# radixsorth/PorousFreezeThaw

Hardware: AMD Instinct MI355X
Metric: Mcells·RK-steps/s at 400³ grid, 1/2/4/8 MI355X; % HBM roofline (higher is better)
Workload: dtype f64; 1 GPU; 400^3 default Params: 200x200x400 cells, Z-slab split 1-way (200x200x400 on rank 0); grid_nodes=400, literal_cube=False, calc_mode=0, cells=16000000, parallelism=zslab1, gl_static=False, kz=auto, tile=1, recompute=True, accepted_steps_total=2981, self_exchange=False, service_callback=False, gl_store_skipped=True, pair_kernels=True, gated_steps=0, gate_misses=0

## Files before the change

porousfreezethaw_amd/csrc/pft_kernels.hip:

```cpp
#include "pft_slab.h"

#include "pft_cosh.h"
#include "pft_ic_ops.h"
#include "pft_tanh.h"

#pragma clang fp contract(off)

__thread char g_err[256];

int fail(hipError_t e, const char* what)
{
  snprintf(g_err, sizeof(g_err), "%s: %s", what, hipGetErrorString(e));
  (void)hipGetLastError();
  return -(int)e - 1000;
}


struct Col {
  double c, xm, xp, ym, yp, zm, zp;
};

__device__ __forceinline__ double lam_of(const pft_consts& c, double p, double g)
{
  return g * c.lam_g + (1.0 - g) * (p * c.lam_i + (1.0 - p) * c.lam_w);
// ... 430 lines not shown

template <int STAGE, int MODE, bool GLS>
__global__ __launch_bounds__(PFT_BLOCK) void merson_stage(StageArgs a, pft_consts c)
{
  const int lin = xcd_remap(blockIdx.x, a.ntile * a.nchunk);
  const int tile = lin % a.ntile, chunk = lin / a.ntile;
  const int cell = tile * PFT_BLOCK + threadIdx.x;
  const bool active = cell < a.plane;
  const int cc = active ? cell : a.plane - 1;
  const int j = cc / a.n1, i = cc - j * a.n1;
  const int kb = a.k_begin + chunk * a.kz;
  const int ke = min(kb + a.kspan, a.k_end);

  const int oxm = i > 0 ? -1 : 0, oxp = i < a.n1 - 1 ? 1 : 0;
  const int oym = j > 0 ? -a.n1 : 0, oyp = j < a.n2 - 1 ? a.n1 : 0;

  const double* fin[3] = {a.in, a.in + a.fs, GLS ? a.x + 2 * a.fs : a.in + 2 * a.fs};

  double m = 0.0;
  bool nf = false;
  double zm[3], zc[3], zp[3], zn[3], nb[3][4], nn[3][4];
  if (kb < ke) {
    const long o0 = (long)(kb + 1) * a.plane + cc;
#pragma unroll
    for (int q = 0; q < 3; ++q) {
      zc[q] = fin[q][o0];
      zm[q] = (kb == 0 && !a.has_below) ? zc[q] : fin[q][o0 - a.plane];
      zp[q] = (kb == a.n3 - 1 && !a.has_above) ? zc[q] : fin[q][o0 + a.plane];
      nb[q][0] = fin[q][o0 + oxm];
      nb[q][1] = fin[q][o0 + oxp];
      nb[q][2] = fin[q][o0 + oym];
      nb[q][3] = fin[q][o0 + oyp];
    }
  }
  for (int k = kb; k < ke; ++k) {
    const long o = (long)(k + 1) * a.plane + cc;
    const bool top = (k == a.n3 - 1) && !a.has_above;
    double xv[3], k1v[3], k3v[3], k4v[3];
    if (STAGE >= 1) {
#pragma unroll
      for (int q = 0; q < 3; ++q) {
        if (GLS && q == 2) continue;
        xv[q] = a.x[q * a.fs + o];
        if (STAGE >= 2) k1v[q] = a.k1[q * a.fs + o];
        if (STAGE >= 4) k3v[q] = a.k3[q * a.fs + o];
        if (STAGE >= 5) k4v[q] = a.k4[q * a.fs + o];
      }
    }
    if (k + 1 < ke) {
      const long o1 = o + a.plane;
      const bool top2 = (k + 1 == a.n3 - 1) && !a.has_above;
#pragma unroll
      for (int q = 0; q < 3; ++q) {
        nn[q][0] = fin[q][o1 + oxm];
        nn[q][1] = fin[q][o1 + oxp];
        nn[q][2] = fin[q][o1 + oym];
        nn[q][3] = fin[q][o1 + oyp];
        zn[q] = top2 ? 0.0 : fin[q][o1 + a.plane];
      }
    }
    Col col[3];
#pragma unroll
    for (int q = 0; q < 3; ++q) {
      col[q].c = zc[q];
      col[q].xm = nb[q][0];
      col[q].xp = nb[q][1];
      col[q].ym = nb[q][2];
      col[q].yp = nb[q][3];
      col[q].zm = zm[q];
      col[q].zp = top ? zc[q] : zp[q];
    }
    if (top) col[0].zp = a.T_top;
    double du = 0.0, dp = 0.0;
    const double un = a.noise ? zc[0] + a.noise[(long)k * a.plane + cc] : zc[0];
    rhs_cell<MODE>(c, col[0], col[1], col[2], un, du, dp);
    if (active) {
      if (STAGE == 0) {
        a.kout[o] = du;
        a.kout[a.fs + o] = dp;
        a.kout[2 * a.fs + o] = 0.0;
      } else {
#pragma unroll
        for (int q = 0; q < 3; ++q) {
          if (GLS && q == 2) continue;
          const double K = q == 0 ? du : (q == 1 ? dp : 0.0);
          const long e = q * a.fs + o;
          if (STAGE == 1) {
            a.kout[e] = K;
            a.out[e] = K * a.coef + xv[q];
          } else if (STAGE == 2) {
            a.out[e] = (k1v[q] + K) * a.coef + xv[q];
          } else if (STAGE == 3) {
            a.kout[e] = K;
            a.out[e] = (k1v[q] + 3.0 * K) * a.coef + xv[q];
          } else if (STAGE == 4) {
            a.kout[e] = K;
            a.out[e] = (0.5 * k1v[q] - 1.5 * k3v[q] + 2.0 * K) * a.h + xv[q];
          } else if (STAGE == 5) {
            const double em = q == 0 ? a.em0 : (q == 1 ? a.em1 : a.em2);
            const double ev = em * fabs(0.2 * k1v[q] - 0.9 * k3v[q] + 0.8 * k4v[q] - 0.1 * K);
            if (ev > m) m = ev;
            nf |= !isfinite(ev);
            a.out[e] = xv[q] + a.coef * (0.5 * (k1v[q] + K) + 2.0 * k4v[q]);
          }
        }
      }
    }
#pragma unroll
    for (int q = 0; q < 3; ++q) {
      zm[q] = zc[q];
      zc[q] = zp[q];
      zp[q] = zn[q];
#pragma unroll
      for (int d = 0; d < 4; ++d) nb[q][d] = nn[q][d];
    }
  }

  if (STAGE == 5) {
    __shared__ double red[PFT_BLOCK / 64];
    __shared__ int rnf[PFT_BLOCK / 64];
#pragma unroll
    for (int off = 32; off > 0; off >>= 1) {
      const double o = __shfl_xor(m, off, 64);
      if (o > m) m = o;
    }
    const int anynf = __any(nf);
    const int w = threadIdx.x >> 6;
    if ((threadIdx.x & 63) == 0) {
      red[w] = m;
      rnf[w] = anynf;
    }
    __syncthreads();
    if (threadIdx.x == 0) {
      double bm = red[0];
      int bnf = rnf[0];
      for (int k = 1; k < PFT_BLOCK / 64; ++k) {
        if (red[k] > bm) bm = red[k];
        bnf |= rnf[k];
      }
      if (bm > 0.0) atomicMax(a.eps_bits, (unsigned long long)__double_as_longlong(bm));
      if (bnf) atomicOr(a.nonfinite, 1u);
    }
  }
}


typedef double dbl2 __attribute__((ext_vector_type(2)));

#define PFT_FUSED_LF 680

__device__ __forceinline__ dbl2 ld2(const double* p) { return *reinterpret_cast<const dbl2*>(p); }
__device__ __forceinline__ void st2(double* p, dbl2 v) { *reinterpret_cast<dbl2*>(p) = v; }


struct Ops {
  dbl2 x, k1, k2, k3, k4;
};

template <int STAGE, bool GLS>
__device__ __forceinline__ void load_ops(const StageArgs& a, int q, long o, Ops& r)
{
  r.x = ld2(a.x + q * a.fs + o);
  if (GLS && q == 2) return;
  if (q == 2) {
    constexpr dbl2 z = {0.0, 0.0};
    r.k1 = z; r.k2 = z; r.k3 = z; r.k4 = z;
    return;
  }
  if (STAGE >= 2 && STAGE != 3) r.k1 = ld2(a.k1 + q * a.fs + o);
  if (STAGE == 3) r.k2 = ld2(a.k2 + q * a.fs + o);
  if (STAGE >= 4) r.k3 = ld2(a.k3 + q * a.fs + o);
  if (STAGE == 5) r.k4 = ld2(a.k4 + q * a.fs + o);
}

template <int STAGE, bool GLS>
__device__ __forceinline__ dbl2 stage_in(const StageArgs& a, int q, const Ops& r)
{
  if (STAGE <= 1 || (GLS && q == 2)) return r.x;
  dbl2 v;
#pragma unroll
  for (int s = 0; s < 2; ++s) {
    if (STAGE == 2) v[s] = r.k1[s] * a.cin + r.x[s];
    if (STAGE == 3) v[s] = r.k2[s] * a.cin + r.x[s];
    if (STAGE == 4) v[s] = (r.k1[s] + 3.0 * r.k3[s]) * a.cin + r.x[s];
    if (STAGE == 5) v[s] = (0.5 * r.k1[s] - 1.5 * r.k3[s] + 2.0 * r.k4[s]) * a.cin + r.x[s];
  }
  return v;
}

template <bool GLS>
__device__ __forceinline__ void keep5(int q, const Ops& r, dbl2& x, dbl2& k1, dbl2& k4, dbl2& E)
{
  x = r.x;
  if (q == 2) return;
  k1 = r.k1;
  k4 = r.k4;
#pragma unroll
  for (int s = 0; s < 2; ++s) E[s] = 0.2 * r.k1[s] - 0.9 * r.k3[s] + 0.8 * r.k4[s];
}

template <int STAGE, int MODE, bool GLS>
__global__ __launch_bounds__(PFT_FBLOCK) __attribute__((amdgpu_waves_per_eu(STAGE >= 1 ? 2 : 3))) void merson_fused(StageArgs a, pft_consts c)
{
  const int WX = a.gwx, TY = a.gty, TX = 2 * WX, LW = TX + 4, LH = TY + 2, NH = LW + 2 * TY;
  __shared__ __attribute__((aligned(16))) double lds[2][3][PFT_FUSED_LF];

  unsigned long long gw0 = 0, gw1 = 0, gw2 = 0;
  if (a.gate) {
    gw0 = __hip_atomic_load(a.gate, __ATOMIC_RELAXED, __HIP_MEMORY_SCOPE_AGENT);
    gw1 = a.gate[1];
    gw2 = a.gate[2];
  }
  if (STAGE == 1 && (a.npart > 0 || a.gdev) && (int)blockIdx.x == a.nbw + a.nint) {
    unsigned long long m = 0, f = 0;
    if (a.npart > 0) eps_part_load(a.part, a.npart, m, f);
    if (a.gate) {
      if (gw0 != a.gseq) return;
      a.dt = __longlong_as_double((long long)gw1);
      a.dh = __longlong_as_double((long long)gw2);
    }
    if (a.npart > 0) eps_part_publish(m, f, a.pub, &m, &f);
    if (a.gdev && threadIdx.x == 0) gate_decide(a, a.dt, a.dh, m, (int)f, a.npart > 0);
    return;
  }
  const int ntx = (a.n1 + TX - 1) / TX;
  const bool bw = (int)blockIdx.x < a.nbw;
  const int lin = bw ? xcd_remap(blockIdx.x, a.nbw) : xcd_remap(blockIdx.x - a.nbw, a.nint);
  const int tile = lin % a.ntile, cq = lin / a.ntile;
  const int chunk = bw ? (a.bends ? (cq ? a.nchunk - 1 : 0) : cq) : a.c0 + cq;
  const bool bshort = bw && !a.bends;
  const int x0 = (tile % ntx) * TX, y0 = (tile / ntx) * TY;
  const int tt = min((int)threadIdx.x, WX * TY - 1);
  const int tx = tt % WX, ty = tt / WX;
  const int i0 = x0 + 2 * tx, j = y0 + ty;
  const bool active = (i0 < a.n1) && (j < a.n2) && (int)threadIdx.x < WX * TY;
  const long po = (long)(j < a.n2 ? j : a.n2 - 1) * a.n1 + (i0 < a.n1 ? i0 : a.n1 - 2);
  const int kb = bshort ? chunk * (a.n3 - 2) : a.k_begin + chunk * a.kz;
  const int ke = bshort ? kb + 2 : min(kb + a.kspan, a.k_end);
  const int lo = (ty + 1) * LW + 2 + 2 * tx;

  const int t = threadIdx.x;
  const bool hact = t < 3 * NH;
  const int hf = hact ? t / NH : 0, h = hact ? t % NH : 0;
  int hr, hcp;
  if (h < LW / 2) { hr = 0; hcp = h; }
  else if (h < LW) { hr = LH - 1; hcp = h - LW / 2; }
  else { const int q = h - LW; hr = 1 + q / 2; hcp = (q & 1) ? LW / 2 - 1 : 0; }
  const int hi = x0 - 2 + 2 * hcp, hj = y0 + hr - 1;
  const long hp = (long)(hj < 0 ? 0 : (hj >= a.n2 ? a.n2 - 1 : hj)) * a.n1 +
                  (hi < 0 ? 0 : (hi >= a.n1 ? a.n1 - 2 : hi));
  const int hl = hr * LW + 2 * hcp;
  const int xma = i0 - 2 < 0 ? 1 : 0, xpa = i0 + 2 >= a.n1 ? 1 : 0;

  double m = 0.0;
  bool nf = false;
  dbl2 zm[3], zc[3], zp[3];
  constexpr bool FLUX = MODE != 10 && MODE != 11;
  constexpr bool DEEP = STAGE >= 1 && STAGE <= 4;
  Ops pn[3], ph;
  FaceT fz[2];
  constexpr bool SUM2 = STAGE == 2;
  dbl2 s2c[3], s2n[3];
  dbl2 cx[3], ck1[3], ck4[3], cE[3], nx[3], nk1[3], nk4[3], nE[3];
  int cur = 0;
  const long o0 = (long)(kb + 1) * a.plane + po;
  const bool wlo = kb == 0 && !a.has_below;
  const long ob = wlo ? o0 : o0 - a.plane;
  Ops cop[3], bop[3], hop;
  if (kb < ke) {
#pragma unroll
    for (int q = 0; q < 3; ++q) load_ops<STAGE, GLS>(a, q, o0, cop[q]);
#pragma unroll
    for (int q = 0; q < 3; ++q) load_ops<STAGE, GLS>(a, q, ob, bop[q]);
    load_ops<STAGE, GLS>(a, hf, (long)(kb + 1) * a.plane + hp, hop);
  }
  if (a.gate) {
    if (gw0 != a.gseq) return;
    const double gt = __longlong_as_double((long long)gw1), gh = __longlong_as_double((long long)gw2);
    gate_scalars<STAGE>(a, c, gt, gh);
    a.dt = gt;
    a.dh = gh;
  }
  if (kb < ke) {
#pragma unroll
    for (int q = 0; q < 3; ++q) {
      zc[q] = stage_in<STAGE, GLS>(a, q, cop[q]);
      if constexpr (SUM2) s2c[q] = cop[q].k1;
      if (STAGE == 5) keep5<GLS>(q, cop[q], cx[q], ck1[q], ck4[q], cE[q]);
      zm[q] = wlo ? zc[q] : stage_in<STAGE, GLS>(a, q, bop[q]);
      st2(&lds[0][q][lo], zc[q]);
    }
    if (hact) st2(&lds[0][hf][hl], stage_in<STAGE, GLS>(a, hf, hop));
    if constexpr (DEEP) {
      if (!((kb == a.n3 - 1) && !a.has_above)) {
#pragma unroll
        for (int q = 0; q < 3; ++q) load_ops<STAGE, GLS>(a, q, o0 + a.plane, pn[q]);
      }
      if (hact && kb + 1 < ke) load_ops<STAGE, GLS>(a, hf, (long)(kb + 2) * a.plane + hp, ph);
    }
#pragma unroll
    for (int s = 0; s < 2; ++s)
      fz[s] = face_of(c, zm[1][s], zm[2][s], zm[0][s], zc[1][s], zc[2][s], zc[0][s], FLUX);
    __syncthreads();
  }
  for (int k = kb; k < ke; ++k) {
    const long o = (long)(k + 1) * a.plane + po;
    const bool top = (k == a.n3 - 1) && !a.has_above;
    const bool more = k + 1 < ke;
    if (!top) {
#pragma unroll
      for (int q = 0; q < 3; ++q) {
        if constexpr (DEEP) {
          zp[q] = stage_in<STAGE, GLS>(a, q, pn[q]);
          if constexpr (SUM2) s2n[q] = pn[q].k1;
        } else {
          Ops nop;
          load_ops<STAGE, GLS>(a, q, o + a.plane, nop);
          zp[q] = stage_in<STAGE, GLS>(a, q, nop);
          if constexpr (SUM2) s2n[q] = nop.k1;
          if (STAGE == 5) keep5<GLS>(q, nop, nx[q], nk1[q], nk4[q], nE[q]);
        }
      }
    }
    dbl2 hv = {0.0, 0.0};
    if (more) {
#pragma unroll
      for (int q = 0; q < 3; ++q) st2(&lds[cur ^ 1][q][lo], zp[q]);
      if (hact) {
        if constexpr (DEEP) {
          hv = stage_in<STAGE, GLS>(a, hf, ph);
        } else {
          Ops tmp;
          load_ops<STAGE, GLS>(a, hf, (long)(k + 2) * a.plane + hp, tmp);
          hv = stage_in<STAGE, GLS>(a, hf, tmp);
        }
      }
    }
    if constexpr (DEEP) {
      if (more) {
        if (!((k + 1 == a.n3 - 1) && !a.has_above)) {
#pragma unroll
          for (int q = 0; q < 3; ++q) load_ops<STAGE, GLS>(a, q, o + 2 * a.plane, pn[q]);
        }
        if (hact && k + 2 < ke) load_ops<STAGE, GLS>(a, hf, (long)(k + 3) * a.plane + hp, ph);
      }
    }
    if (top) {
#pragma unroll
      for (int q = 1; q < 3; ++q) zp[q] = zc[q];
      zp[0] = dbl2{a.T_top, a.T_top};
    }
    double du[2], dp[2];
    FaceT fx;
    dbl2 ym2[3], yp2[3];
#pragma unroll
    for (int q = 0; q < 3; ++q) {
      ym2[q] = ld2(&lds[cur][q][lo - LW]);
      yp2[q] = ld2(&lds[cur][q][lo + LW]);
    }
#pragma unroll
    for (int s = 0; s < 2; ++s) {
      Col col[3];
#pragma unroll
      for (int q = 0; q < 3; ++q) {
        const double* L = lds[cur][q];
        const double cen = zc[q][s];
        col[q].c = cen;
        col[q].xm = s == 0 ? L[lo - 1 - xma] : zc[q][0];
        col[q].xp = s == 0 ? zc[q][1] : L[lo + 2 + xpa];
        col[q].ym = ym2[q][s];
        col[q].yp = yp2[q][s];
        col[q].zm = zm[q][s];
        col[q].zp = zp[q][s];
      }
      const double un = a.noise ? zc[0][s] + a.noise[(long)k * a.plane + po + s] : zc[0][s];
      const FaceT fxm =
          s == 0 ? face_of(c, col[1].xm, col[2].xm, col[0].xm, col[1].c, col[2].c, col[0].c, FLUX) : fx;
      FaceT fzp;
      rhs_cell_f<MODE>(c, col[0], col[1], col[2], un, fxm, fz[s], fx, fzp, du[s], dp[s]);
      fz[s] = fzp;
    }
    if (more && hact) st2(&lds[cur ^ 1][hf][hl], hv);
    if (active) {
#pragma unroll
      for (int q = 0; q < 3; ++q) {
        if (q == 2 && STAGE != 0 && (GLS || STAGE <= 4)) continue;
        const dbl2 K = q == 0 ? dbl2{du[0], du[1]} : (q == 1 ? dbl2{dp[0], dp[1]} : dbl2{0.0, 0.0});
        const long e = q * a.fs + o;
        if (SUM2) {
          dbl2 S;
          const dbl2 k1c = s2c[q];
#pragma unroll
          for (int s = 0; s < 2; ++s) S[s] = k1c[s] + K[s];
          st2(a.kout + e, S);
        } else if (STAGE <= 4) {
          st2(a.kout + e, K);
        } else {
          constexpr dbl2 zero2 = {0.0, 0.0};
          const bool z2 = q == 2;
          const dbl2 ox = cx[q], ok1 = z2 ? zero2 : ck1[q], ok4 = z2 ? zero2 : ck4[q];
          dbl2 oE = cE[q];
          if (z2) {
#pragma unroll
            for (int s = 0; s < 2; ++s) oE[s] = 0.2 * 0.0 - 0.9 * 0.0 + 0.8 * 0.0;
          }
          dbl2 r;
#pragma unroll
          for (int s = 0; s < 2; ++s) {
            const double em = q == 0 ? a.em0 : (q == 1 ? a.em1 : a.em2);
            const double ev = em * fabs(oE[s] - 0.1 * K[s]);
            if (ev > m) m = ev;
            nf |= !isfinite(ev);
            r[s] = ox[s] + a.coef * (0.5 * (ok1[s] + K[s]) + 2.0 * ok4[s]);
          }
          if (!(q == 2 && a.gl_keep)) st2(a.out + e, r);
        }
      }
    }
    __syncthreads();
    cur ^= 1;
#pragma unroll
    for (int q = 0; q < 3; ++q) {
      zm[q] = zc[q];
      zc[q] = zp[q];
      if constexpr (SUM2) s2c[q] = s2n[q];
      if (STAGE == 5) { cx[q] = nx[q]; ck1[q] = nk1[q]; ck4[q] = nk4[q]; cE[q] = nE[q]; }
    }
  }

  if (STAGE == 5) {
    __shared__ double red[PFT_FBLOCK / 64];
    __shared__ int rnf[PFT_FBLOCK / 64];
#pragma unroll
    for (int off = 32; off > 0; off >>= 1) {
      const double ov = __shfl_xor(m, off, 64);
      if (ov > m) m = ov;
    }
    const int anynf = __any(nf);
    const int w = threadIdx.x >> 6;
    if ((threadIdx.x & 63) == 0) {
      red[w] = m;
      rnf[w] = anynf;
    }
    __syncthreads();
    if (threadIdx.x == 0) {
      double bm = red[0];
      int bnf = rnf[0];
      for (int q = 1; q < PFT_FBLOCK / 64; ++q) {
        if (red[q] > bm) bm = red[q];
        bnf |= rnf[q];
      }
      if (a.part) eps_store_part(a.part, bm, bnf);
      else eps_arrive(bm, bnf, a.shards, a.eps_bits, a.nonfinite, a.pub, a.pub_count);
    }
  }
  if (bw) {
    asm volatile("s_waitcnt vmcnt(0)" ::: "memory");
    __syncthreads();
    if (threadIdx.x == 0) {
      __builtin_amdgcn_fence(__ATOMIC_RELEASE, "");
      __hip_atomic_fetch_add(a.bdone, 1ULL, __ATOMIC_RELAXED, __HIP_MEMORY_SCOPE_AGENT);
    }
  }
}

#define PFT_PBLOCK 512
#define PFT_PAIR_NEX 16
#define PFT_PAIR_PADP 2
#define PFT_PAIR_H 532
#define PFT_PAIR_HB 488
#define PFT_PAIR_MIN_CELLS_PER_CU 2560

struct PairArgs {
  const double* x;
  const double* k1;
  const double* k3;
  double* out;
  const double* noise;
  unsigned long long* eps_bits;
  unsigned int* nonfinite;
  unsigned long long* pub;
  unsigned int* pub_count;
  EpsShard* shards;
  unsigned long long* part;
  long fs;
  int n1, n2, n3, plane;
  int has_below, has_above;
  int k_begin, k_end, kz, ntile, nchunk, ntx;
  int kspan;
  int nbw, bends, c0, nint;
  unsigned long long* bdone;
  int tx, ty;
  double T_topA, T_topB;
  double cinA, cinB;
  double coef;
  double em0, em1;
  double glA, glB, glX, evgl;
  int gl_keep;
};
static constexpr unsigned PFT_PAIR_COFF =
    (unsigned)((sizeof(PairArgs) + alignof(pft_consts) - 1) / alignof(pft_consts) * alignof(pft_consts));

#if defined(__HIP_DEVICE_COMPILE__)
typedef const __attribute__((address_space(4))) char* pft_kptr;
#define PFT_PAIR_BIND(A, C)                                                                  \
  pft_kptr kq_##A = kbase;                                                                  \
  asm volatile("" : "+s"(kq_##A));                                                          \
  const PairArgs& A = *(const __attribute__((address_space(4))) PairArgs*)kq_##A;           \
  const pft_consts& C = *(const __attribute__((address_space(4))) pft_consts*)(kq_##A + PFT_PAIR_COFF)
#else
#define PFT_PAIR_BIND(A, C) \
  const PairArgs& A = a;    \
  const pft_consts& C = c
#endif

struct PairRaw {
  dbl2 x[3], k1[2], k3[2];
};

__device__ __forceinline__ dbl2 ldb(const double* base, unsigned bo)
{
  return *reinterpret_cast<const dbl2*>(reinterpret_cast<const char*>(base) + bo);
}
__device__ __forceinline__ void stb(double* base, unsigned bo, dbl2 v)
{
  *reinterpret_cast<dbl2*>(reinterpret_cast<char*>(base) + bo) = v;
}

template <int SA, bool GL = true>
__device__ __forceinline__ void pair_load(const PairArgs& a, unsigned bo, PairRaw& r)
{
#pragma unroll
  for (int q = 0; q < (GL ? 3 : 2); ++q) r.x[q] = ldb(a.x + q * a.fs, bo);
#pragma unroll
  for (int q = 0; q < 2; ++q) {
    r.k1[q] = ldb(a.k1 + q * a.fs, bo);
    if (SA == 4) r.k3[q] = ldb(a.k3 + q * a.fs, bo);
  }
}

template <int SA, bool GLX>
__device__ __forceinline__ dbl2 pair_in_A(const PairArgs& a, int q, const PairRaw& r)
{
  if (q == 2) {
    if (GLX) return r.x[2];
    return dbl2{a.glA + r.x[2][0], a.glA + r.x[2][1]};
  }
  const dbl2 k1 = r.k1[q < 2 ? q : 0];
  const dbl2 k3 = r.k3[q < 2 ? q : 0];
  dbl2 v;
#pragma unroll
  for (int s = 0; s < 2; ++s) {
    if (SA == 2) v[s] = k1[s] * a.cinA + r.x[q][s];
    else v[s] = (k1[s] + 3.0 * k3[s]) * a.cinA + r.x[q][s];
  }
  return v;
}

template <int SA, bool GLX>
__device__ __forceinline__ dbl2 pair_in_B(const PairArgs& a, int q, const PairRaw& r, dbl2 KA)
{
  if (q == 2) {
    if (GLX) return r.x[2];
    return dbl2{a.glB + r.x[2][0], a.glB + r.x[2][1]};
  }
  const dbl2 k1 = r.k1[q < 2 ? q : 0];
  const dbl2 k3 = r.k3[q < 2 ? q : 0];
  dbl2 v;
#pragma unroll
  for (int s = 0; s < 2; ++s) {
    if (SA == 2) v[s] = (k1[s] + KA[s]) * a.cinB + r.x[q][s];
    else v[s] = (0.5 * k1[s] - 1.5 * k3[s] + 2.0 * KA[s]) * a.cinB + r.x[q][s];
  }
  return v;
}

#define PFT_PAIR_OPN 400
struct PairLds {
  __device__ static __forceinline__ dbl2 ld(const double* L, int p) { return ld2(L + 2 * p); }
  __device__ static __forceinline__ void st(double* L, int p, dbl2 v) { st2(L + 2 * p, v); }
  __device__ static __forceinline__ double cell(const double* L, int p, int s) { return L[2 * p + s]; }
};

template <int MODE, int LWP>
__device__ __forceinline__ void pair_rhs(const pft_consts& c, const double* L0, const double* L1, const double* L2,
                                         int p, int xmc, int xpc, const dbl2* zm, const dbl2* zc, const dbl2* zp,
                                         const double* nz, FaceT* fz, double* du, double* dp)
{
  constexpr bool FLUX = MODE != 10 && MODE != 11;
  using LD = PairLds;
  const double* L[3] = {L0, L1, L2};
  dbl2 ym2[3], yp2[3];
#pragma unroll
  for (int q = 0; q < 3; ++q) {
    ym2[q] = LD::ld(L[q], p - LWP);
    yp2[q] = LD::ld(L[q], p + LWP);
  }
  FaceT fx;
#pragma unroll
  for (int s = 0; s < 2; ++s) {
    Col col[3];
#pragma unroll
    for (int q = 0; q < 3; ++q) {
      const double cen = zc[q][s];
      col[q].c = cen;
      col[q].xm = s == 0 ? LD::cell(L[q], p - 1, xmc) : zc[q][0];
      col[q].xp = s == 0 ? zc[q][1] : LD::cell(L[q], p + 1, xpc);
      col[q].ym = ym2[q][s];
      col[q].yp = yp2[q][s];
      col[q].zm = zm[q][s];
      col[q].zp = zp[q][s];
    }
    const double un = nz ? zc[0][s] + nz[s] : zc[0][s];
    const FaceT fxm =
        s == 0 ? face_of(c, col[1].xm, col[2].xm, col[0].xm, col[1].c, col[2].c, col[0].c, FLUX) : fx;
    FaceT fzp;
    rhs_cell_f<MODE>(c, col[0], col[1], col[2], un, fxm, fz[s], fx, fzp, du[s], dp[s]);
    fz[s] = fzp;
  }
}

__device__ __forceinline__ void pair_pos(int v, int bw, int ty, int& px, int& py)
{
  const int wp2 = bw + 2;
  if (v < ty * wp2) {
    py = 2 + v / wp2;
    px = v % wp2;
    return;
  }
  v -= ty * wp2;
  if (v < 2 * wp2) {
    py = v < wp2 ? 1 : ty + 2;
    px = v < wp2 ? v : v - wp2;
    return;
  }
  v -= 2 * wp2;
  py = v < wp2 ? 0 : ty + 3;
  px = v < wp2 ? v : v - wp2;
}

template <int N>
using pft_ic = std::integral_constant<int, N>;

#pragma clang diagnostic push
#pragma clang diagnostic ignored "-Warray-bounds"
template <int SA, int MODE, bool GLX, int LWP>
__global__ __launch_bounds__(PFT_PBLOCK) __attribute__((amdgpu_waves_per_eu(2))) void merson_pair(PairArgs a,
                                                                                                   pft_consts c)
{
  constexpr bool FLUX = MODE != 10 && MODE != 11;
  constexpr dbl2 zero2 = {0.0, 0.0};
  using LD = PairLds;
#if defined(__HIP_DEVICE_COMPILE__)
  const pft_kptr kbase = (pft_kptr)__builtin_amdgcn_kernarg_segment_ptr();
#endif
  constexpr bool GLB = GLX;
  constexpr bool OPL = SA == 4 && GLB;
  constexpr int NBQ = GLB ? 2 : 3;
  __shared__ __attribute__((aligned(16))) double lA[3][3][2 * PFT_PAIR_H];
  __shared__ __attribute__((aligned(16))) double lB[3][NBQ][2 * PFT_PAIR_HB];
  __shared__ __attribute__((aligned(16))) dbl2 lO[OPL ? 6 : 1][OPL ? PFT_PAIR_OPN : 1];
  __shared__ unsigned lXa[PFT_PAIR_NEX];

  const int TX = a.tx, TY = a.ty, WP2 = TX / 2 + 2, NPOS = WP2 * (TY + 4);
  const bool bw = (int)blockIdx.x < a.nbw;
  const int lin = bw ? xcd_remap(blockIdx.x, a.nbw) : xcd_remap(blockIdx.x - a.nbw, a.nint);
  const int tile = lin % a.ntile, cq = lin / a.ntile;
  const int chunk = bw ? (a.bends ? (cq ? a.nchunk - 1 : 0) : cq) : a.c0 + cq;
  const bool bshort = bw && !a.bends;
  const int x0 = (tile % a.ntx) * TX, y0 = (tile / a.ntx) * TY;
  const int tt = min((int)threadIdx.x, NPOS - 1);
  int px, py;
  if (LWP == 22 && NPOS > PFT_PBLOCK) {
    pair_pos(tt, TX / 2, TY, px, py);
  } else {
    px = tt % WP2;
    py = tt / WP2;
  }
  const int pi = x0 - 2 + 2 * px, pj = y0 - 2 + py;
  const int ai = pi < 0 ? 0 : (pi >= a.n1 ? a.n1 - 2 : pi);
  const int aj = pj < 0 ? 0 : (pj >= a.n2 ? a.n2 - 1 : pj);
  auto mir = [&](int col) -> bool { const int c0 = x0 - 2 + 2 * col; return c0 < 0 || c0 >= a.n1; };
  const int pxa = (ai - x0 + 2) / 2;
  const int xmcA = mir(pxa - 1) ? 0 : 1, xpcA = mir(pxa + 1) ? 1 : 0;
  const int xmcB = mir(px - 1) ? 0 : 1, xpcB = mir(px + 1) ? 1 : 0;
  const unsigned apo = (unsigned)(aj * a.n1 + ai);
  auto pbo = [&](int m) -> unsigned { return ((unsigned)(m + 2) * (unsigned)a.plane + apo) * 8u; };
  const int posA = PFT_PAIR_PADP + py * LWP + px;
  const int posB = PFT_PAIR_PADP + (py - 1) * LWP + px;
  const int actA = PFT_PAIR_PADP + (aj - y0 + 2) * LWP + (ai - x0 + 2) / 2;
  const bool isA = py >= 1 && py <= TY + 2;
  const bool isB = (int)threadIdx.x < NPOS && px >= 1 && px <= TX / 2 && py >= 2 && py <= TY + 1 &&
                   pi < a.n1 && pj < a.n2;
  const int ob = (py - 2) * (TX / 2) + px - 1;
  auto nex = [&](const PairArgs& A) { return (A.tx / 2 + 2) * (A.ty + 4) - PFT_PBLOCK; };
  const int wid = __builtin_amdgcn_readfirstlane((int)threadIdx.x >> 6);
  auto lane = [&]() {
    int l;
    asm volatile("v_mbcnt_lo_u32_b32 %0, -1, 0\n\tv_mbcnt_hi_u32_b32 %0, -1, %0" : "=v"(l));
    return l;
  };
  auto is_x = [&](const PairArgs& A) { return LWP == 22 && wid == PFT_PBLOCK / 64 - 1 && lane() >= 64 - nex(A); };
  auto px_x = [&](const PairArgs& A) { return lane() - 64 + (A.tx / 2 + 2); };
  auto apo_x = [&](const PairArgs& A) { return lXa[lane() - (64 - nex(A))]; };
  auto pos_x = [&](const PairArgs& A) { return PFT_PAIR_PADP + (A.ty + 3) * LWP + px_x(A); };
  auto pboe = [&](const PairArgs& A, int m) -> unsigned { return ((unsigned)(m + 2) * (unsigned)A.plane + apo_x(A)) * 8u; };
  auto xload = [&](const PairArgs& A, int m, PairRaw& r) { pair_load<SA>(A, pboe(A, m), r); };
  auto xstore = [&](const PairArgs& A, int slot, const PairRaw& r) {
    const int pe = pos_x(A);
#pragma unroll
    for (int q = 0; q < 3; ++q) LD::st(lA[slot][q], pe, pair_in_A<SA, GLX>(A, q, r));
  };

  const int kb = bshort ? chunk * (a.n3 - 2) : a.k_begin + chunk * a.kz;
  const int ke = bshort ? kb + 2 : min(kb + a.kspan, a.k_end);
  const int n3 = a.n3;
  const bool wlo = !a.has_below, whi = !a.has_above;
  const int mA0 = kb > 0 ? kb - 1 : (wlo ? 0 : -1);
  const int mA1 = ke < n3 ? ke : (whi ? n3 - 1 : n3);
  const int mlast = min(mA1 + 1, whi ? n3 - 1 : n3 + 1);
  const int mfirst = wlo ? 0 : -2;

  double m = 0.0;
  bool nf = false;
  PairRaw R[3];
  dbl2 KA[3][2];
  constexpr bool ZREG = SA == 2;
  dbl2 IA[3][3];
  dbl2 glm = zero2;
  FaceT fzA[2], fzB[2];

  if (is_x(a)) {
    const int ajx = min(y0 - 2 + a.ty + 3, a.n2 - 1);
    const int aix = min(max(x0 - 2 + 2 * px_x(a), 0), a.n1 - 2);
    lXa[(int)threadIdx.x - (PFT_PBLOCK - nex(a))] = (unsigned)(ajx * a.n1 + aix);
  }
  if (kb < ke) {
    dbl2 ia0[3], iam[3];
    pair_load<SA>(a, pbo(mA0), R[0]);
    if (mA0 > mfirst) {
      PairRaw t;
      pair_load<SA>(a, pbo(mA0 - 1), t);
#pragma unroll
      for (int q = 0; q < 3; ++q) {
        iam[q] = pair_in_A<SA, GLX>(a, q, t);
        LD::st(lA[2][q], posA, iam[q]);
        if (ZREG) IA[2][q] = iam[q];
      }
    }
#pragma unroll
    for (int q = 0; q < 3; ++q) {
      ia0[q] = pair_in_A<SA, GLX>(a, q, R[0]);
      LD::st(lA[0][q], posA, ia0[q]);
      if (ZREG) IA[0][q] = ia0[q];
      if (mA0 == mfirst) {
        iam[q] = ia0[q];
        LD::st(lA[2][q], posA, ia0[q]);
        if (ZREG) IA[2][q] = ia0[q];
      }
    }
#pragma unroll
    for (int s = 0; s < 2; ++s) fzA[s] = face_of(c, iam[1][s], iam[2][s], iam[0][s], ia0[1][s], ia0[2][s], ia0[0][s], FLUX);
    if (is_x(a)) {
      PairRaw t;
      if (mA0 > mfirst) {
        pair_load<SA>(a, pboe(a, mA0 - 1), t);
#pragma unroll
        for (int q = 0; q < 3; ++q) LD::st(lA[2][q], pos_x(a), pair_in_A<SA, GLX>(a, q, t));
      }
      pair_load<SA>(a, pboe(a, mA0), t);
#pragma unroll
      for (int q = 0; q < 3; ++q) {
        const dbl2 v = pair_in_A<SA, GLX>(a, q, t);
        LD::st(lA[0][q], pos_x(a), v);
        if (mA0 == mfirst) LD::st(lA[2][q], pos_x(a), v);
      }
      if (mA0 + 1 <= mlast) xload(a, mA0 + 1, R[0]);
    }
    if (mA0 + 1 <= mlast) pair_load<SA>(a, pbo(mA0 + 1), R[1]);
    KA[2][0] = KA[2][1] = zero2;
    __syncthreads();
  }

  auto step = [&](auto ph, auto st, int mm, PairRaw& rc, PairRaw& rn, PairRaw& rnn) -> bool {
    constexpr int PH = decltype(ph)::value;
    constexpr int ST = decltype(st)::value;
    constexpr bool SDY = ST != 0;
    constexpr int sA = PH, sAm = (PH + 2) % 3, sAp = (PH + 1) % 3;
#if defined(__HIP_DEVICE_COMPILE__)
    if (SDY) asm volatile("" : "+s"(mm));
#endif
    {
      PFT_PAIR_BIND(A0, C0);
      (void)C0;
      if (GLB) glm = ZREG ? IA[sAp][2] : LD::ld(lA[sAp][2], posA);
// ... 851 lines not shown
}

int pft_slab_upload_host(pft_slab* s, int which, const double* host_padded)
{
  if (which == PFT_BUF_X || which == PFT_BUF_XN) s->gl_keep = 0;
  int rc = ensure_staging(s);
  if (rc) return rc;
  HIPCHK(hipMemcpyAsync(s->staging, host_padded, sizeof(double) * 3 * (size_t)s->S, hipMemcpyHostToDevice,
                        s->stream));
  pack_kernel<<<2048, 256, 0, s->stream>>>(s->staging, s->buf[which], s->d.n1, s->d.n2, s->d.n3, s->fs, s->S);
  HIPCHK(hipGetLastError());
  return slab_wait(s, nullptr, "upload");
}

int pft_slab_download_host(pft_slab* s, int which, double* host_padded)
{
  int rc = ensure_staging(s);
  if (rc) return rc;
  HIPCHK(hipMemcpyAsync(s->staging, host_padded, sizeof(double) * 3 * (size_t)s->S, hipMemcpyHostToDevice,
                        s->stream));
  unpack_kernel<<<2048, 256, 0, s->stream>>>(s->buf[which], s->staging, s->d.n1, s->d.n2, s->d.n3, s->fs, s->S);
  HIPCHK(hipGetLastError());
  HIPCHK(hipMemcpyAsync(host_padded, s->staging, sizeof(double) * 3 * (size_t)s->S, hipMemcpyDeviceToHost,
                        s->stream));
  return slab_wait(s, nullptr, "download");
}

}

template <int STAGE, int MODE, bool GLS>
static int kernel_occupancy(int kind)
{
  static int cache[2] = {0, 0};
  int& n = cache[kind == KFUSED];
  if (n) return n;
  const void* f = kind == KFUSED ? (const void*)merson_fused<STAGE, MODE, GLS>
                                 : (const void*)merson_stage<STAGE, MODE, GLS>;
  int b = 0;
  if (hipOccupancyMaxActiveBlocksPerMultiprocessor(&b, f, kind == KFUSED ? PFT_FBLOCK : PFT_BLOCK, 0) != hipSuccess || b < 1) b = 1;
  n = b;
  return n;
}

static int stage_occupancy(int stage, int mode, int gls, int kind)
{
  return with_stage(stage, [&](auto st) {
    return with_mode(mode, [&](auto m) {
      return with_bool(gls, [&](auto g) {
        return kernel_occupancy<decltype(st)::value, decltype(m)::value, decltype(g)::value>(kind);
      });
    });
  });
}

static void launch_stage(int stage, int mode, int gls, int kind, dim3 g, hipStream_t st, const StageArgs& a,
                         const pft_consts& c)
{
  with_stage(stage, [&](auto sv) {
    with_mode(mode, [&](auto mv) {
      with_bool(gls, [&](auto gv) {
        constexpr int STAGE = decltype(sv)::value, MODE = decltype(mv)::value;
        constexpr bool GLS = decltype(gv)::value;
        if (kind == KFUSED) {
          merson_fused<STAGE, MODE, GLS><<<g, PFT_FBLOCK, 0, st>>>(a, c);
        } else {
          merson_stage<STAGE, MODE, GLS><<<g, PFT_BLOCK, 0, st>>>(a, c);
        }
      });
    });
  });
}

extern "C" {

static bool fused_geometry_ok(int wx, int ty)
{
  return wx >= 4 && ty >= 1 && wx * ty <= PFT_FBLOCK && 3 * (2 * wx + 4 + 2 * ty) <= PFT_FBLOCK &&
         (2 * wx + 4) * (ty + 2) <= PFT_FUSED_LF;
}

static double fused_geometry(int n1, int n2, int* wx_out, int* ty_out)
{
  const int np = n1 / 2;
  double best = -1.0;
  int bw = 32, bt = 8;
  for (int wx = 16; wx <= 40; ++wx) {
    int ty = PFT_FBLOCK / wx;
    while (ty > 1 && !fused_geometry_ok(wx, ty)) --ty;
    if (!fused_geometry_ok(wx, ty)) continue;
    const long lanes = (long)((np + wx - 1) / wx) * ((n2 + ty - 1) / ty) * PFT_FBLOCK;
    const double eff = (double)np * n2 / (double)lanes;
    if (eff >= best - 0.005) {
      if (eff > best) best = eff;
      bw = wx;
      bt = ty;
    }
  }
  *wx_out = bw;
  *ty_out = bt;
  return best;
}

static double slab_fgeo(const pft_slab* cs, int* wx, int* ty)
{
  pft_slab* s = const_cast<pft_slab*>(cs);
  if (!s->fgeo_valid) {
    s->fgeo_eff = fused_geometry(s->d.n1, s->d.n2, &s->fgeo_wx, &s->fgeo_ty);
    s->fgeo_valid = 1;
  }
  *wx = s->fgeo_wx;
  *ty = s->fgeo_ty;
  return s->fgeo_eff;
}

static int kz_memo_get(const pft_slab* s, int slot, long key)
{
  return s->kz_key[slot] == key + 1 ? s->kz_val[slot] : 0;
}
static void kz_memo_put(pft_slab* s, int slot, long key, int kz)
{
  s->kz_key[slot] = key + 1;
  s->kz_val[slot] = kz;
}

static int chunk_kz(pft_slab* s, int slot, int occ, long ntile, int nplanes, int min_nch = 1)
{
  const long key = ((long)occ << 52) ^ ((long)s->cu_reserved << 44) ^ (ntile << 24) ^ (long)nplanes;
  int kz = kz_memo_get(s, slot, key);
  if (kz) return kz;
  int best_nch = 1;
  double best_cost = -1.0;
  if (min_nch > nplanes) min_nch = nplanes;
  for (int nch = min_nch; nch <= nplanes; ++nch) {
    const int k = (nplanes + nch - 1) / nch;
    if (nch > min_nch && k == (nplanes + nch - 2) / (nch - 1)) continue;
    if ((nplanes + k - 1) / k < min_nch) continue;
    if (min_nch >= 3 && (k < 2 || nplanes - ((nplanes + k - 1) / k - 1) * k < 2)) continue;
    const long nb = ntile * ((nplanes + k - 1) / k);
    const int ncu = s->n_cu - s->cu_reserved;
    const long per_cu = (nb + ncu - 1) / ncu;
    const double rounds = occ <= 2 ? (double)((per_cu + occ - 1) / occ) : std::max(1.0, (double)per_cu / occ);
    const double cost = rounds * (k + 2);
    if (best_cost < 0.0 || cost < 0.95 * best_cost) { best_cost = cost; best_nch = nch; }
  }
  if (best_cost < 0.0) best_nch = std::max(1, nplanes);
  kz = (nplanes + best_nch - 1) / best_nch;
  kz_memo_put(s, slot, key, kz);
  return kz;
}

static int slab_kind(const pft_slab* s)
{
  if (s->d.n1 % 2 != 0 || s->tile_wx == 0 || !s->recompute) return KCACHE;
  if (s->tile_wx == 1) {
    int wx, ty;
    if (slab_fgeo(s, &wx, &ty) < 0.7) return KCACHE;
  }
  return KFUSED;
}

int pft_slab_stage_output(const pft_slab* s, int stage)
{
  static const int aux_out[6] = {-1, PFT_BUF_A0, PFT_BUF_A1, PFT_BUF_A0, PFT_BUF_A1, PFT_BUF_XN};
  static const int rc_out[6] = {-1, PFT_BUF_K1, PFT_BUF_A0 , PFT_BUF_K3, PFT_BUF_K4, PFT_BUF_XN};
  if (stage < 1 || stage > 5) return -2;
  return slab_kind(s) == KFUSED ? rc_out[stage] : aux_out[stage];
}

int pft_slab_tile_geometry(const pft_slab* s, int stage, int* wx, int* ty)
{
  const int kind = slab_kind(s);
  const bool auto_tile = s->tile_wx == 1 || s->tile_wx == 2;
  if (kind == KCACHE) {
    *wx = 0;
    *ty = 0;
  } else if (auto_tile) {
    slab_fgeo(s, wx, ty);
  } else {
    *wx = s->tile_wx;
    *ty = PFT_FBLOCK / *wx;
  }
  return kind;
}

int pft_slab_launch_geometry(const pft_slab* s, int stage, int* nwg, int* kz, int* ntile)
{
  if (stage < 1 || stage > 5 || !s->launch_nwg[stage]) return -2;
  *nwg = s->launch_nwg[stage];
  *kz = s->launch_kz[stage];
  *ntile = s->launch_ntile[stage];
  return s->launch_bnd[stage] ? 1 : 0;
}

int pft_xcd_remap(int b, int n) { return xcd_remap(b, n); }

int pft_slab_eps_route(const pft_slab* s)
{
  if (!s->launch_nwg[5]) return -2;
  return s->launch_part ? 1 : 0;
}

int pft_slab_stage_fields(const pft_slab* s, int stage)
{
  if (stage < 1 || stage > 6) return -2;
  if (s->d.gl_static) return 2;
  if (slab_kind(s) == KFUSED && stage != 5) return 2;
  if (stage == 5 && pft_slab_get_gl_keep(s) && slab_kind(s) == KFUSED) return 2;
  return 3;
}

static int defer_arm(pft_slab* s, long nwg, int j, unsigned long long** part, long cap_nwg = 0)
{
  if (std::max(nwg, cap_nwg) > s->part_cap) {
    if (s->part) HIPCHK(hipFree(s->part));
    s->part = nullptr;
    s->part_cap = 0;
    const long cap = std::max(std::max(nwg, cap_nwg), 4096L);
    HIPCHK(hipMalloc((void**)&s->part, 16 * (size_t)cap));
    s->part_cap = cap;
  }
  s->defer_n = (int)nwg;
  s->defer_slot = j;
  *part = s->part;
  return 0;
}

static int run_stage(pft_slab* s, int stage, const double* in, double* kout, double* out, double t_stage,
                     double coef, double h, int k_begin, int k_end, int gls, int kind)
{
  const int mode = s->d.calc_mode;
  if (mode != 0 && mode != 1 && mode != 2 && mode != 10 && mode != 11) return -2;
  const bool bnd = k_begin == PFT_K_BOUNDARY || k_begin == PFT_K_BOUNDARY2;
  const int bdepth = k_begin == PFT_K_BOUNDARY2 ? 2 : 1;
  bool ends = k_begin == PFT_K_ENDS_FIRST;
  const bool inl = k_begin == PFT_K_INLINE || ends;
  if (inl && (kind != KFUSED || !s->bdone || s->d.n3 < 5 || s->gate_use_seq)) return -2;
  if (bnd || inl) {
    k_begin = 0;
    k_end = s->d.n3;
  }
  if (k_begin < 0) k_begin = 0;
  if (k_end < 0 || k_end > s->d.n3) k_end = s->d.n3;
  if (k_end <= k_begin) return 0;
  StageArgs a;
  memset(&a, 0, sizeof(a));
  a.in = in;
  a.x = s->buf[PFT_BUF_X];
  a.k1 = s->buf[PFT_BUF_K1];
  a.k2 = s->buf[PFT_BUF_A0];
  a.k3 = s->buf[PFT_BUF_K3];
  a.k4 = s->buf[PFT_BUF_K4];
  a.kout = kout;
  a.out = out;
  a.noise = s->noise;
  a.eps_bits = s->scratch;
  a.shards = s->eps_shards + (bnd ? PFT_EPS_SHARDS : 0);
  a.nonfinite = (unsigned int*)(s->scratch + 1);
  a.fs = s->fs;
  a.n1 = s->d.n1;
  a.n2 = s->d.n2;
  a.n3 = s->d.n3;
  a.plane = s->plane;
  a.has_below = s->d.has_below;
  a.has_above = s->d.has_above;
  a.k_begin = k_begin;
  a.k_end = k_end;
  const bool auto_tile = s->tile_wx == 1 || s->tile_wx == 2;
  if (kind == KFUSED) {
    if (auto_tile) {
      slab_fgeo(s, &a.gwx, &a.gty);
    } else {
      a.gwx = s->tile_wx;
      a.gty = PFT_FBLOCK / s->tile_wx;
    }
    if (!fused_geometry_ok(a.gwx, a.gty)) return -2;
    a.ntile = ((s->d.n1 + 2 * a.gwx - 1) / (2 * a.gwx)) * ((s->d.n2 + a.gty - 1) / a.gty);
  } else {
    a.ntile = (s->plane + PFT_BLOCK - 1) / PFT_BLOCK;
  }
  if (ends) {
    const int n3 = s->d.n3;
    const int occ = stage_occupancy(stage, mode, gls, kind);
    const int kz = s->kz > 0 ? s->kz : chunk_kz(s, 14, occ, a.ntile, n3, 3);
    const int nch = (n3 + kz - 1) / kz;
    if (kz < 2 || nch < 3 || n3 - (nch - 1) * kz < 2) ends = false;
  }
  if (inl) {
    k_begin = ends ? 0 : 2;
    k_end = ends ? s->d.n3 : s->d.n3 - 2;
    a.k_begin = k_begin;
    a.k_end = k_end;
  }
  const int nplanes = k_end - k_begin;
  if (s->kz > 0) {
    a.kz = s->kz;
  } else if (ends) {
    a.kz = chunk_kz(s, 14, stage_occupancy(stage, mode, gls, kind), a.ntile, nplanes, 3);
  } else {
    const int occ = stage_occupancy(stage, mode, gls, kind);
    a.kz = chunk_kz(s, stage + 6 * (gls ? 1 : 0), occ, a.ntile, nplanes);
  }
  a.nchunk = (nplanes + a.kz - 1) / a.kz;
  a.kspan = a.kz;
  if (bnd) {
    a.kz = std::max(1, s->d.n3 - bdepth);
    a.kspan = bdepth;
// ... 1375 lines not shown
```

Baseline: 20360 Mcells·steps/s.

## Unroll fused stage-1 z-loop by three with rotating registers and 32-bit offsets

Restructures the fused Merson stage kernel's z-plane loop into a lambda step that, for stage 1 with low modes, runs a 3-way unrolled steady-state with register rotation (no copying of zm/zc/zp) and a triple-buffered LDS. Global loads and stores switch to scalar base plus 32-bit unsigned byte offset addressing with inline-asm hints to keep the base in SGPRs, aiming to cut address arithmetic. Stage-1 occupancy hint moves from 2 to 3 waves per EU. It adds a guard falling back to the cache kernel when a plane's byte offset would overflow 32 bits, and it raises LDS use and code size for the unrolled variant.

```diff
diff --git a/porousfreezethaw_amd/csrc/pft_kernels.hip b/porousfreezethaw_amd/csrc/pft_kernels.hip
--- a/porousfreezethaw_amd/csrc/pft_kernels.hip
+++ b/porousfreezethaw_amd/csrc/pft_kernels.hip
@@ -606,25 +606,57 @@
 __device__ __forceinline__ dbl2 ld2(const double* p) { return *reinterpret_cast<const dbl2*>(p); }
 __device__ __forceinline__ void st2(double* p, dbl2 v) { *reinterpret_cast<dbl2*>(p) = v; }
 
+__device__ __forceinline__ dbl2 ldb(const double* base, unsigned bo)
+{
+  return *reinterpret_cast<const dbl2*>(reinterpret_cast<const char*>(base) + bo);
+}
+__device__ __forceinline__ void stb(double* base, unsigned bo, dbl2 v)
+{
+  *reinterpret_cast<dbl2*>(reinterpret_cast<char*>(base) + bo) = v;
+}
+#if defined(__HIP_DEVICE_COMPILE__)
+#define PFT_GLOBAL __attribute__((address_space(1)))
+#else
+#define PFT_GLOBAL
+#endif
+template <bool UB = true>
+__device__ __forceinline__ dbl2 ldu(const double* base, unsigned bo)
+{
+  if (!UB) return ldb(base, bo);
+#if defined(__HIP_DEVICE_COMPILE__)
+  asm("" : "+s"(base));
+#endif
+  return *reinterpret_cast<const PFT_GLOBAL dbl2*>((const PFT_GLOBAL char*)base + bo);
+}
+template <bool UB = true>
+__device__ __forceinline__ void stu(double* base, unsigned bo, dbl2 v)
+{
+  if (!UB) return stb(base, bo, v);
+#if defined(__HIP_DEVICE_COMPILE__)
+  asm("" : "+s"(base));
+#endif
+  *reinterpret_cast<PFT_GLOBAL dbl2*>((PFT_GLOBAL char*)base + bo) = v;
+}
+
 
 struct Ops {
   dbl2 x, k1, k2, k3, k4;
 };
 
-template <int STAGE, bool GLS>
-__device__ __forceinline__ void load_ops(const StageArgs& a, int q, long o, Ops& r)
-{
-  r.x = ld2(a.x + q * a.fs + o);
+template <int STAGE, bool GLS, bool UB = true>
+__device__ __forceinline__ void load_ops(const StageArgs& a, int q, long o, unsigned bo, Ops& r)
+{
+  r.x = ldu<UB>(a.x + q * a.fs + o, bo);
   if (GLS && q == 2) return;
   if (q == 2) {
     constexpr dbl2 z = {0.0, 0.0};
     r.k1 = z; r.k2 = z; r.k3 = z; r.k4 = z;
     return;
   }
-  if (STAGE >= 2 && STAGE != 3) r.k1 = ld2(a.k1 + q * a.fs + o);
-  if (STAGE == 3) r.k2 = ld2(a.k2 + q * a.fs + o);
-  if (STAGE >= 4) r.k3 = ld2(a.k3 + q * a.fs + o);
-  if (STAGE == 5) r.k4 = ld2(a.k4 + q * a.fs + o);
+  if (STAGE >= 2 && STAGE != 3) r.k1 = ldu<UB>(a.k1 + q * a.fs + o, bo);
+  if (STAGE == 3) r.k2 = ldu<UB>(a.k2 + q * a.fs + o, bo);
+  if (STAGE >= 4) r.k3 = ldu<UB>(a.k3 + q * a.fs + o, bo);
+  if (STAGE == 5) r.k4 = ldu<UB>(a.k4 + q * a.fs + o, bo);
 }
 
 template <int STAGE, bool GLS>
@@ -653,11 +685,16 @@
   for (int s = 0; s < 2; ++s) E[s] = 0.2 * r.k1[s] - 0.9 * r.k3[s] + 0.8 * r.k4[s];
 }
 
+template <int N>
+using pft_ic = std::integral_constant<int, N>;
+
+constexpr bool fused_unrolled(int stage, int mode, bool gls) { return stage == 1 && mode <= 2; }
+
 template <int STAGE, int MODE, bool GLS>
-__global__ __launch_bounds__(PFT_FBLOCK) __attribute__((amdgpu_waves_per_eu(STAGE >= 1 ? 2 : 3))) void merson_fused(StageArgs a, pft_consts c)
+__global__ __launch_bounds__(PFT_FBLOCK) __attribute__((amdgpu_waves_per_eu(STAGE >= 2 ? 2 : 3))) void merson_fused(StageArgs a, pft_consts c)
 {
   const int WX = a.gwx, TY = a.gty, TX = 2 * WX, LW = TX + 4, LH = TY + 2, NH = LW + 2 * TY;
-  __shared__ __attribute__((aligned(16))) double lds[2][3][PFT_FUSED_LF];
+  __shared__ __attribute__((aligned(16))) double lds[fused_unrolled(STAGE, MODE, GLS) ? 3 : 2][3][PFT_FUSED_LF];
 
   unsigned long long gw0 = 0, gw1 = 0, gw2 = 0;
   if (a.gate) {
@@ -689,6 +726,8 @@
   const int i0 = x0 + 2 * tx, j = y0 + ty;
   const bool active = (i0 < a.n1) && (j < a.n2) && (int)threadIdx.x < WX * TY;
   const long po = (long)(j < a.n2 ? j : a.n2 - 1) * a.n1 + (i0 < a.n1 ? i0 : a.n1 - 2);
+  unsigned pob = (unsigned)po * 8u;
+  auto ppl = [&](int m) -> long { return (long)(m + 1) * a.plane; };
   const int kb = bshort ? chunk * (a.n3 - 2) : a.k_begin + chunk * a.kz;
   const int ke = bshort ? kb + 2 : min(kb + a.kspan, a.k_end);
   const int lo = (ty + 1) * LW + 2 + 2 * tx;
@@ -703,30 +742,31 @@
   const int hi = x0 - 2 + 2 * hcp, hj = y0 + hr - 1;
   const long hp = (long)(hj < 0 ? 0 : (hj >= a.n2 ? a.n2 - 1 : hj)) * a.n1 +
                   (hi < 0 ? 0 : (hi >= a.n1 ? a.n1 - 2 : hi));
+  const unsigned hpb = (unsigned)hp * 8u;
   const int hl = hr * LW + 2 * hcp;
   const int xma = i0 - 2 < 0 ? 1 : 0, xpa = i0 + 2 >= a.n1 ? 1 : 0;
 
   double m = 0.0;
   bool nf = false;
-  dbl2 zm[3], zc[3], zp[3];
   constexpr bool FLUX = MODE != 10 && MODE != 11;
+  constexpr bool UNR = fused_unrolled(STAGE, MODE, GLS);
+  dbl2 Z[3][3];
   constexpr bool DEEP = STAGE >= 1 && STAGE <= 4;
   Ops pn[3], ph;
   FaceT fz[2];
   constexpr bool SUM2 = STAGE == 2;
-  dbl2 s2c[3], s2n[3];
-  dbl2 cx[3], ck1[3], ck4[3], cE[3], nx[3], nk1[3], nk4[3], nE[3];
-  int cur = 0;
-  const long o0 = (long)(kb + 1) * a.plane + po;
+  dbl2 S2[3][3];
+  struct Keep5 {
+    dbl2 x[3], k1[3], k4[3], E[3];
+  } K5[3];
   const bool wlo = kb == 0 && !a.has_below;
-  const long ob = wlo ? o0 : o0 - a.plane;
   Ops cop[3], bop[3], hop;
   if (kb < ke) {
 #pragma unroll
-    for (int q = 0; q < 3; ++q) load_ops<STAGE, GLS>(a, q, o0, cop[q]);
-#pragma unroll
-    for (int q = 0; q < 3; ++q) load_ops<STAGE, GLS>(a, q, ob, bop[q]);
-    load_ops<STAGE, GLS>(a, hf, (long)(kb + 1) * a.plane + hp, hop);
+    for (int q = 0; q < 3; ++q) load_ops<STAGE, GLS, UNR>(a, q, ppl(kb), pob, cop[q]);
+#pragma unroll
+    for (int q = 0; q < 3; ++q) load_ops<STAGE, GLS, UNR>(a, q, ppl(wlo ? kb : kb - 1), pob, bop[q]);
+    load_ops<STAGE, GLS, false>(a, hf, ppl(kb), hpb, hop);
   }
   if (a.gate) {
     if (gw0 != a.gseq) return;
@@ -736,11 +776,12 @@
     a.dh = gh;
   }
   if (kb < ke) {
+    dbl2 (&zm)[3] = Z[2], (&zc)[3] = Z[0];
 #pragma unroll
     for (int q = 0; q < 3; ++q) {
       zc[q] = stage_in<STAGE, GLS>(a, q, cop[q]);
-      if constexpr (SUM2) s2c[q] = cop[q].k1;
-      if (STAGE == 5) keep5<GLS>(q, cop[q], cx[q], ck1[q], ck4[q], cE[q]);
+      if constexpr (SUM2) S2[0][q] = cop[q].k1;
+      if (STAGE == 5) keep5<GLS>(q, cop[q], K5[0].x[q], K5[0].k1[q], K5[0].k4[q], K5[0].E[q]);
       zm[q] = wlo ? zc[q] : stage_in<STAGE, GLS>(a, q, bop[q]);
       st2(&lds[0][q][lo], zc[q]);
     }
@@ -748,55 +789,61 @@
     if constexpr (DEEP) {
       if (!((kb == a.n3 - 1) && !a.has_above)) {
 #pragma unroll
-        for (int q = 0; q < 3; ++q) load_ops<STAGE, GLS>(a, q, o0 + a.plane, pn[q]);
+        for (int q = 0; q < 3; ++q) load_ops<STAGE, GLS, UNR>(a, q, ppl(kb + 1), pob, pn[q]);
       }
-      if (hact && kb + 1 < ke) load_ops<STAGE, GLS>(a, hf, (long)(kb + 2) * a.plane + hp, ph);
+      if (hact && kb + 1 < ke) load_ops<STAGE, GLS, false>(a, hf, ppl(kb + 1), hpb, ph);
     }
 #pragma unroll
     for (int s = 0; s < 2; ++s)
       fz[s] = face_of(c, zm[1][s], zm[2][s], zm[0][s], zc[1][s], zc[2][s], zc[0][s], FLUX);
     __syncthreads();
   }
-  for (int k = kb; k < ke; ++k) {
-    const long o = (long)(k + 1) * a.plane + po;
-    const bool top = (k == a.n3 - 1) && !a.has_above;
-    const bool more = k + 1 < ke;
+
+  auto step = [&](auto phv, auto stv, int k, int cur, int nxt) __attribute__((always_inline)) -> bool {
+    constexpr int PH = decltype(phv)::value, PN = (PH + 1) % 3, PM = (PH + 2) % 3;
+    constexpr bool SDY = decltype(stv)::value != 0;
+#if defined(__HIP_DEVICE_COMPILE__)
+    if (UNR) asm volatile("" : "+s"(k));
+    if (UNR) asm volatile("" : "+v"(pob));
+#endif
+    dbl2 (&zm)[3] = Z[PM], (&zc)[3] = Z[PH], (&zp)[3] = Z[PN];
+    const bool top = !SDY && (k == a.n3 - 1) && !a.has_above;
+    const bool more = SDY || k + 1 < ke;
     if (!top) {
 #pragma unroll
       for (int q = 0; q < 3; ++q) {
         if constexpr (DEEP) {
           zp[q] = stage_in<STAGE, GLS>(a, q, pn[q]);
-          if constexpr (SUM2) s2n[q] = pn[q].k1;
+          if constexpr (SUM2) S2[PN][q] = pn[q].k1;
         } else {
           Ops nop;
-          load_ops<STAGE, GLS>(a, q, o + a.plane, nop);
+          load_ops<STAGE, GLS, UNR>(a, q, ppl(k + 1), pob, nop);
           zp[q] = stage_in<STAGE, GLS>(a, q, nop);
-          if constexpr (SUM2) s2n[q] = nop.k1;
-          if (STAGE == 5) keep5<GLS>(q, nop, nx[q], nk1[q], nk4[q], nE[q]);
+          if (STAGE == 5) keep5<GLS>(q, nop, K5[PN].x[q], K5[PN].k1[q], K5[PN].k4[q], K5[PN].E[q]);
         }
       }
     }
     dbl2 hv = {0.0, 0.0};
     if (more) {
 #pragma unroll
-      for (int q = 0; q < 3; ++q) st2(&lds[cur ^ 1][q][lo], zp[q]);
-      if (hact) {
+      for (int q = 0; q < 3; ++q) st2(&lds[nxt][q][lo], zp[q]);
+      if (SDY || hact) {
         if constexpr (DEEP) {
           hv = stage_in<STAGE, GLS>(a, hf, ph);
         } else {
           Ops tmp;
-          load_ops<STAGE, GLS>(a, hf, (long)(k + 2) * a.plane + hp, tmp);
+          load_ops<STAGE, GLS, false>(a, hf, ppl(k + 1), hpb, tmp);
           hv = stage_in<STAGE, GLS>(a, hf, tmp);
         }
       }
     }
     if constexpr (DEEP) {
       if (more) {
-        if (!((k + 1 == a.n3 - 1) && !a.has_above)) {
-#pragma unroll
-          for (int q = 0; q < 3; ++q) load_ops<STAGE, GLS>(a, q, o + 2 * a.plane, pn[q]);
+        if (SDY || !((k + 1 == a.n3 - 1) && !a.has_above)) {
+#pragma unroll
+          for (int q = 0; q < 3; ++q) load_ops<STAGE, GLS, UNR>(a, q, ppl(k + 2), pob, pn[q]);
         }
-        if (hact && k + 2 < ke) load_ops<STAGE, GLS>(a, hf, (long)(k + 3) * a.plane + hp, ph);
+        if (SDY || (hact && k + 2 < ke)) load_ops<STAGE, GLS, false>(a, hf, ppl(k + 2), hpb, ph);
       }
     }
     if (top) {
@@ -827,33 +874,36 @@
         col[q].zm = zm[q][s];
         col[q].zp = zp[q][s];
       }
-      const double un = a.noise ? zc[0][s] + a.noise[(long)k * a.plane + po + s] : zc[0][s];
+      const double un = (!SDY && a.noise) ? zc[0][s] + a.noise[(long)k * a.plane + po + s] : zc[0][s];
       const FaceT fxm =
           s == 0 ? face_of(c, col[1].xm, col[2].xm, col[0].xm, col[1].c, col[2].c, col[0].c, FLUX) : fx;
       FaceT fzp;
       rhs_cell_f<MODE>(c, col[0], col[1], col[2], un, fxm, fz[s], fx, fzp, du[s], dp[s]);
       fz[s] = fzp;
     }
-    if (more && hact) st2(&lds[cur ^ 1][hf][hl], hv);
+    if (more && hact) st2(&lds[nxt][hf][hl], hv);
     if (active) {
+#if defined(__HIP_DEVICE_COMPILE__)
+      if (UNR) asm volatile("" : "+v"(pob));
+#endif
 #pragma unroll
       for (int q = 0; q < 3; ++q) {
         if (q == 2 && STAGE != 0 && (GLS || STAGE <= 4)) continue;
         const dbl2 K = q == 0 ? dbl2{du[0], du[1]} : (q == 1 ? dbl2{dp[0], dp[1]} : dbl2{0.0, 0.0});
-        const long e = q * a.fs + o;
+        const long e = q * a.fs + ppl(k);
         if (SUM2) {
           dbl2 S;
-          const dbl2 k1c = s2c[q];
+          const dbl2 k1c = S2[PH][q];
 #pragma unroll
           for (int s = 0; s < 2; ++s) S[s] = k1c[s] + K[s];
-          st2(a.kout + e, S);
+          stu<UNR>(a.kout + e, pob, S);
         } else if (STAGE <= 4) {
-          st2(a.kout + e, K);
+          stu<UNR>(a.kout + e, pob, K);
         } else {
           constexpr dbl2 zero2 = {0.0, 0.0};
           const bool z2 = q == 2;
-          const dbl2 ox = cx[q], ok1 = z2 ? zero2 : ck1[q], ok4 = z2 ? zero2 : ck4[q];
-          dbl2 oE = cE[q];
+          const dbl2 ox = K5[PH].x[q], ok1 = z2 ? zero2 : K5[PH].k1[q], ok4 = z2 ? zero2 : K5[PH].k4[q];
+          dbl2 oE = K5[PH].E[q];
           if (z2) {
 #pragma unroll
             for (int s = 0; s < 2; ++s) oE[s] = 0.2 * 0.0 - 0.9 * 0.0 + 0.8 * 0.0;
@@ -867,18 +917,32 @@
             nf |= !isfinite(ev);
             r[s] = ox[s] + a.coef * (0.5 * (ok1[s] + K[s]) + 2.0 * ok4[s]);
           }
-          if (!(q == 2 && a.gl_keep)) st2(a.out + e, r);
+          if (!(q == 2 && a.gl_keep)) stu<UNR>(a.out + e, pob, r);
         }
       }
     }
     __syncthreads();
-    cur ^= 1;
-#pragma unroll
-    for (int q = 0; q < 3; ++q) {
-      zm[q] = zc[q];
-      zc[q] = zp[q];
-      if constexpr (SUM2) s2c[q] = s2n[q];
-      if (STAGE == 5) { cx[q] = nx[q]; ck1[q] = nk1[q]; ck4[q] = nk4[q]; cE[q] = nE[q]; }
+    return more;
+  };
+
+  if (kb < ke) {
+    int k = kb;
+    if constexpr (UNR) {
+      const int ksteady = a.noise ? -(1 << 30) : ke - 5;
+      for (; k <= ksteady; k += 3) {
+        step(pft_ic<0>{}, pft_ic<1>{}, k, 0, 1);
+        step(pft_ic<1>{}, pft_ic<1>{}, k + 1, 1, 2);
+        step(pft_ic<2>{}, pft_ic<1>{}, k + 2, 2, 0);
+      }
+    }
+    for (int cur = 0; step(pft_ic<0>{}, pft_ic<0>{}, k, cur, cur ^ 1); ++k, cur ^= 1) {
+#pragma unroll
+      for (int q = 0; q < 3; ++q) {
+        Z[2][q] = Z[0][q];
+        Z[0][q] = Z[1][q];
+        if constexpr (SUM2) S2[0][q] = S2[1][q];
+      }
+      if (STAGE == 5) K5[0] = K5[1];
     }
   }
 
@@ -972,15 +1036,6 @@
   dbl2 x[3], k1[2], k3[2];
 };
 
-__device__ __forceinline__ dbl2 ldb(const double* base, unsigned bo)
-{
-  return *reinterpret_cast<const dbl2*>(reinterpret_cast<const char*>(base) + bo);
-}
-__device__ __forceinline__ void stb(double* base, unsigned bo, dbl2 v)
-{
-  *reinterpret_cast<dbl2*>(reinterpret_cast<char*>(base) + bo) = v;
-}
-
 template <int SA, bool GL = true>
 __device__ __forceinline__ void pair_load(const PairArgs& a, unsigned bo, PairRaw& r)
 {
@@ -1092,9 +1147,6 @@
   py = v < wp2 ? 0 : ty + 3;
   px = v < wp2 ? v : v - wp2;
 }
-
-template <int N>
-using pft_ic = std::integral_constant<int, N>;
 
 #pragma clang diagnostic push
 #pragma clang diagnostic ignored "-Warray-bounds"
@@ -2252,6 +2304,7 @@
 static int slab_kind(const pft_slab* s)
 {
   if (s->d.n1 % 2 != 0 || s->tile_wx == 0 || !s->recompute) return KCACHE;
+  if ((long)s->plane * 8 >= (1L << 32)) return KCACHE;
   if (s->tile_wx == 1) {
     int wx, ty;
     if (slab_fgeo(s, &wx, &ty) < 0.7) return KCACHE;
```

Result: no change. 20490 Mcells·steps/s (median of 6 runs) (+0.6%).
